# hguo/ftk

Measured on NVIDIA B200. Metric: space_time_simplices_tested_per_sec, higher is better.
Workload: dtype f64+int64

## Files before the change

### ftk_b200/csrc/context.cpp

```cpp
#include <algorithm>
#include <cfloat>
#include <chrono>
#include <cmath>
#include <cstdio>
#include <cstdlib>
#include <cstring>
#include <deque>
#include <string>
#include <thread>
#include <atomic>
#include <vector>

#include <memory>
#include "kernels.h"
#include "online.h"
#include "curves.h"

using namespace ftkb;

namespace {

thread_local std::string g_create_error;

struct Layer {
// ... 593 lines not shown
    c->stats.h2d_bytes += 8 * n;
  }
  return FTKB_OK;
}

static void fill_sweep_geometry(const ftkb_ctx *c, SweepParams &p) {
  p.coords_mode = c->coords_mode;
  p.coords_ncomp = c->coords_ncomp;
  for (int k = 0; k < 6; k++) p.coords_bounds[k] = c->coords_bounds[k];
  p.coords = c->d_coords;
  p.nd = c->n;
  p.sm_count = c->sm_count;
  p.W = c->cfg.dims[0]; p.H = c->cfg.dims[1]; p.D = c->n == 3 ? c->cfg.dims[2] : 1;
  for (int j = 0; j < 3; j++) {
    const bool used = j < c->n;
    p.lb[j] = used ? c->cfg.lb[j] : 0;
    p.ub[j] = used ? c->cfg.ub[j] : 0;
    p.nc[j] = p.ub[j] - p.lb[j] + 1;
    p.vmax[j] = p.ub[j];
    p.voff[j] = 0; p.rank_lb[j] = p.lb[j]; p.rank_nc[j] = p.nc[j];
  }
  for (int j = 0; j < 3; j++)
    p.res_thr[j] = res_threshold_key(c->resolution, c->n == 2 ? (double)(c->cfg.dims[j < 2 ? j : 0] - 1) : 0.5);
  if (c->slab) {
    p.voff[2] = c->cfg.slab_offset;
    p.rank_lb[2] = c->cfg.slab_global_lb;
    p.rank_nc[2] = c->cfg.slab_global_ub - c->cfg.slab_global_lb + 1;
  }
}

static void fused2d_decomposition(const ftkb_ctx *c, SweepParams &p, bool aligned) {
  if (aligned) {
    const int R = SCAN2D_CELL_ROWS;
    p.nsx = std::max(1, (p.W + 7 * 62 - 1) / (7 * 62));
    const int64_t want = std::max<int64_t>(1, (8 * (int64_t)c->sm_count * 3) / p.nsx);
    p.rows = std::max(2 * R, (int)((p.H + want - 1) / want));
    p.rows = (p.rows + R - 1) / R * R;
    p.rows = std::min(p.rows, 64 * R);
  } else {
    p.nsx = std::max(1, (p.W - 1 + 59) / 60);
    int64_t nsy = (2 * (int64_t)c->sm_count * 2 * 8) / p.nsx;
    nsy = std::max<int64_t>(1, std::min<int64_t>(nsy, (p.H + 31) / 32));
    p.rows = (int)((p.H + nsy - 1) / nsy);
  }
  p.nsy = (p.H + p.rows - 1) / p.rows;
  p.nsz = 1;
}

static void fused3d_decomposition(const ftkb_ctx *c, SweepParams &p) {
  p.nsx = (p.W + F3_STRIDE - 1) / F3_STRIDE;
  p.nsy = (p.H + F3_TROWS - 1) / F3_TROWS;
  const int64_t tiles = (int64_t)p.nsx * p.nsy;
  const int64_t slots = 2 * (int64_t)c->sm_count;
  const int64_t nsz = std::max<int64_t>(1, std::min<int64_t>((6 * slots + tiles - 1) / tiles, std::max(1, p.D / 16)));
  p.rows = (int)((p.D + nsz - 1) / nsz);
  p.rows = std::min(p.rows, 63);
  p.nsz = (p.D + p.rows - 1) / p.rows;
}

static void vcells_decomposition(const ftkb_ctx *c, SweepParams &p) {
  if (c->n == 3) { fused3d_decomposition(c, p); return; }
  const int R = VSCAN2D_CELL_ROWS;
  p.nsx = std::max(1, (p.W + 61) / 62);
  const int64_t want = std::max<int64_t>(1, (6 * (int64_t)c->sm_count * 16) / p.nsx);
  p.rows = std::max(2 * R, (int)((p.H + want - 1) / want));
  p.rows = (p.rows + R - 1) / R * R;
  p.nsy = (p.H + p.rows - 1) / p.rows;
// ... 1314 lines not shown
```

### ftk_b200/csrc/kernels.cu

```cuda
#include "kernels.h"

#include <algorithm>
#include <cfloat>
#include <cstdlib>
#include <string>
#include <climits>
#include <cub/device/device_radix_sort.cuh>
#include <cub/device/device_select.cuh>

namespace ftkb {

typedef long long i64;
typedef unsigned long long u64;

__constant__ DeviceMeshTables c_mesh[2];

void upload_mesh_tables(const DeviceMeshTables &t2, const DeviceMeshTables &t3) {
  DeviceMeshTables h[2] = {t2, t3};
  cudaMemcpyToSymbol(c_mesh, h, sizeof(h));
}

constexpr int KEY_ONE = 0x3FF00000;
constexpr int KEY_POISON_EXP = 0x43E00000;

// ... 342 lines not shown
  const int lane = threadIdx.x & 31;
  const i64 warp = (i64)blockIdx.x * (blockDim.x >> 5) + (threadIdx.x >> 5);
  const int sx = (int)(warp % p.nsx), cy = (int)(warp / p.nsx);
  if (cy >= p.nsy) return;
  const int b = sx * 60;
  if (b == 0 || b + 65 > p.W) fused2d_strip<HAS_NEXT, true>(p, b, cy, lane);
  else fused2d_strip<HAS_NEXT, false>(p, b, cy, lane);
}

constexpr int FB_SEG = 68;
constexpr int FB_STRIDE = 62;

__device__ __forceinline__ uint32_t smem_u32(const void *q) { return (uint32_t)__cvta_generic_to_shared(q); }
__device__ __forceinline__ void mbar_init(uint32_t bar, uint32_t count) {
  asm volatile("mbarrier.init.shared::cta.b64 [%0], %1;" ::"r"(bar), "r"(count) : "memory");
}
__device__ __forceinline__ void mbar_expect_tx(uint32_t bar, uint32_t bytes) {
  asm volatile("mbarrier.arrive.expect_tx.shared::cta.b64 _, [%0], %1;" ::"r"(bar), "r"(bytes) : "memory");
}
__device__ __forceinline__ void bulk_g2s(uint32_t dst, const void *src, uint32_t bytes, uint32_t bar) {
  asm volatile("cp.async.bulk.shared::cluster.global.mbarrier::complete_tx::bytes [%0], [%1], %2, [%3];"
               ::"r"(dst), "l"(src), "r"(bytes), "r"(bar) : "memory");
}
__device__ __forceinline__ void mbar_wait(uint32_t bar, uint32_t parity) {
  uint32_t done;
  do {
    asm volatile("{\n\t.reg .pred p;\n\tmbarrier.try_wait.parity.shared::cta.b64 p, [%1], %2;\n\tselp.u32 %0, 1, 0, p;\n\t}"
                 : "=r"(done) : "r"(bar), "r"(parity) : "memory");
  } while (!done);
}
__device__ __forceinline__ void mbar_arrive(uint32_t bar) {
  asm volatile("mbarrier.arrive.shared::cta.b64 _, [%0];" ::"r"(bar) : "memory");
}

__device__ __forceinline__ void tma_load_3d(uint32_t dst, const CUtensorMap *tm, int c0, int c1, int c2, uint32_t bar) {
  asm volatile("cp.async.bulk.tensor.3d.shared::cluster.global.tile.mbarrier::complete_tx::bytes [%0], [%1, {%2, %3, %4}], [%5];"
               ::"r"(dst), "l"(tm), "r"(c0), "r"(c1), "r"(c2), "r"(bar) : "memory");
}

template <int K> struct IC { static constexpr int value = K; };

__device__ __forceinline__ bool elect_one() {
  uint32_t pred;
  asm volatile("{\n\t.reg .pred p;\n\telect.sync _|p, 0xffffffff;\n\tselp.u32 %0, 1, 0, p;\n\t}" : "=r"(pred));
  return pred != 0;
}

__device__ __forceinline__ void res_update4(double &m, float &mf, bool e_in, bool o_in, double dxe, double dye, double dxo, double dyo, double cw, double ch) {
  const double vxe = dxe * cw, vye = dye * ch, vxo = dxo * cw, vyo = dyo * ch;
  if (e_in) {
    if (vxe != 0.0 && fabs(vxe) < fabs(m)) m = vxe;
    if (vye != 0.0 && fabs(vye) < fabs(m)) m = vye;
  }
  if (o_in) {
    if (vxo != 0.0 && fabs(vxo) < fabs(m)) m = vxo;
    if (vyo != 0.0 && fabs(vyo) < fabs(m)) m = vyo;
  }
  mf = fabs(m) < 1e38 ? __double2float_ru(fabs(m)) * 1.000001f : 3.4028234e38f;
}

constexpr int C2_R = 9;
constexpr int C2_NST = 9;
constexpr int C2_CW = 7;
constexpr int C2_SEG = C2_CW * FB_STRIDE + 8;
static_assert(C2_R % 3 == 0 && C2_R == C2_NST && C2_R == SCAN2D_CELL_ROWS, "row window / ring / cell block must stay aligned");

__device__ __forceinline__ size_t cells2d_index(const SweepParams &p, const int strip, const int kb, const int lane) {
  const size_t nblk = (size_t)(p.H / C2_R + 2);
  return ((size_t)strip * nblk + (size_t)kb) * 32u + (size_t)lane;
}

template <int NL>
__device__ __forceinline__ void cells2d_slow_cubes_t(const SweepParams &p, unsigned failmask, const int c0, const int y0, const uint32_t stage) {
  static_assert(2 * C2_R <= 32, "one lane per cube");
  const int W = p.W, H = p.H;
  const int lane = threadIdx.x & 31;
  const float cwf = (float)(W - 1), chf = (float)(H - 1);
  const float nanf_ = __int_as_float(0x7FC00000);
  const int per = 2 * C2_R, total = per * __popc(failmask);
  for (int q0 = 0; q0 < total; q0 += 32) {
    const int qi = q0 + lane;
    const bool live = qi < total;
    const int which = live ? qi / per : 0, within = live ? qi % per : 0;
    const int src = (int)__fns(failmask, 0, which + 1);
    const int r = within >> 1, q = within & 1;
    const int x = c0 + 2 * src + q, y = y0 + r;
    const bool in = live && x >= p.lb[0] && x <= p.ub[0] && y >= p.lb[1] && y <= p.ub[1];
    const int xs[4] = {clampi(x - 1, W), clampi(x, W), clampi(x + 1, W), clampi(x + 2, W)};
    size_t rows_[4];
#pragma unroll
    for (int k = 0; k < 4; k++) rows_[k] = (size_t)W * (size_t)clampi(y - 1 + k, H);
    FRange rx{nanf_, nanf_}, ry{nanf_, nanf_};
#pragma unroll
    for (int L = 0; L < NL; L++) {
      const double *S = p.L[L].S;
      double h[2][4], lo[2], hi[2];
#pragma unroll
      for (int j = 0; j < 2; j++)
#pragma unroll
        for (int k = 0; k < 4; k++) h[j][k] = __ldg(S + rows_[1 + j] + xs[k]);
#pragma unroll
      for (int i = 0; i < 2; i++) { lo[i] = __ldg(S + rows_[0] + xs[1 + i]); hi[i] = __ldg(S + rows_[3] + xs[1 + i]); }
#pragma unroll
      for (int v = 0; v < 4; v++) {
        const int i = v & 1, j = v >> 1;
        if (!in || x + i > p.ub[0] || y + j > p.ub[1]) continue;
        const double dx = h[j][i + 2] - h[j][i];
        const double dy = (j == 0 ? h[1][i + 1] : hi[i]) - (j == 0 ? lo[i] : h[0][i + 1]);
        const float fx = __double2float_rn(dx) * cwf, fy = __double2float_rn(dy) * chf;
        rx = fmerge(rx, FRange{fx, fx}); ry = fmerge(ry, FRange{fy, fy});
      }
    }
    const bool surv = in && !cube_excluded2_f(rx, ry, p.thrp_f, p.thr2_f, p.lim_f);
    const u64 lin = (u64)(x - p.lb[0]) + (u64)p.nc[0] * (u64)(y - p.lb[1]);
    if (stage) stage_survivors(p, stage, surv, lin);
    else append_survivors(p, surv, lin);
  }
}
__device__ __noinline__ void cells2d_slow_cubes(const SweepParams &p, unsigned failmask, const int c0, const int y0, const int nl, const uint32_t stage = 0) {
  if (nl == 1) cells2d_slow_cubes_t<1>(p, failmask, c0, y0, stage);
  else cells2d_slow_cubes_t<2>(p, failmask, c0, y0, stage);
}

__device__ __forceinline__ void cells2d_decide(const SweepParams &p, const FRange ux, const FRange uy, const bool own, const int e, const int y0, const int nl) {
  const bool fail = own && !cube_excluded2_f(ux, uy, p.thrp_f, p.thr2_f, p.lim_f);
  const unsigned fm = __ballot_sync(0xffffffffu, fail);
  if (fm) cells2d_slow_cubes(p, fm, e - 2 * (int)(threadIdx.x & 31), y0, nl);
}

template <bool BORDER, int NPREV, bool TEST>
__device__ __forceinline__ void cells2d_strip(const SweepParams &p, const int c0, const int r0, const int r1, const int lane,
                                              const double *tile , const uint32_t full0, const uint32_t empty0,
                                              const int strip) {
  const int W = p.W, H = p.H, B = p.build_layer;
  const int e = c0 + 2 * lane, o = e + 1;
  const bool e_in = !BORDER || e < W, o_in = !BORDER || o < W, o1_in = !BORDER || o + 1 < W;
  const bool own_cols = lane <= 30 && ((e >= p.lb[0] && e <= p.ub[0]) || (o >= p.lb[0] && o <= p.ub[0]));
  const int jl = r1 + 1;
  const float cwf = (float)(W - 1), chf = (float)(H - 1);
  const bool want_res = p.res_slot[B] != nullptr;
  double rmin = DBL_MAX;
  float rminf = 3.4028234e38f;
  const uint4 *sum_prev = NPREV ? p.sum_in[0] + cells2d_index(p, strip, 0, lane) : nullptr;
  uint4 *sum_out = p.sum_out + cells2d_index(p, strip, 0, lane);

  const double *lane_base = tile + 2 * lane;
  auto centre = [&](const int st, double (&dst)[2]) {
    const double2 t = *reinterpret_cast<const double2 *>(lane_base + st * C2_SEG + 2);
    dst[0] = t.x; dst[1] = t.y;
  };
  auto release = [&](const int st) {
    __syncwarp();
    if (elect_one()) mbar_arrive(empty0 + 8u * st);
  };
  auto finish_block = [&](const int kb, FRange bx, FRange by, const uint4 prevc) {
    bx = fmerge(bx, fshfl_down1(bx));
    by = fmerge(by, fshfl_down1(by));
    sum_out[(size_t)kb * 32u] = make_uint4(__float_as_uint(bx.mn), __float_as_uint(bx.mx), __float_as_uint(by.mn), __float_as_uint(by.mx));
    if (TEST) {
      if (NPREV) {
        bx = fmerge(bx, FRange{__uint_as_float(prevc.x), __uint_as_float(prevc.y)});
        by = fmerge(by, FRange{__uint_as_float(prevc.z), __uint_as_float(prevc.w)});
      }
      const int y0 = kb * C2_R;
      const bool own = own_cols && y0 <= p.ub[1] && y0 + C2_R - 1 >= p.lb[1];
      cells2d_decide(p, bx, by, own, e, y0, NPREV + 1);
    }
  };

  double win[3][2];
  mbar_wait(full0, 0);
  centre(0, win[0]);
  mbar_wait(full0 + 8, 0);
  centre(1, win[1]);
  release(0);
  FRange bx{0.f, 0.f}, by{0.f, 0.f};
  uint4 prevc = make_uint4(0x7FC00000u, 0x7FC00000u, 0x7FC00000u, 0x7FC00000u);

  auto step = [&](auto KC, const int j, const int i) {
    constexpr int K = decltype(KC)::value;
    constexpr int ST_J = (1 + K) % C2_NST, ST_P = (2 + K) % C2_NST;
    double (&m1)[2] = win[K % 3];
    double (&c0v)[2] = win[(K + 1) % 3];
    double (&p1)[2] = win[(K + 2) % 3];
    mbar_wait(full0 + 8u * ST_P, (uint32_t)((i + (2 + K >= C2_NST ? 1 : 0)) & 1));
    centre(ST_P, p1);
    const double *rowj = lane_base + ST_J * C2_SEG;
    double left = rowj[1], right = rowj[4];
    double mid_e = c0v[1];
    if (BORDER) {
      if (e == 0) left = c0v[0];
      if (!o_in) mid_e = c0v[0];
      if (!o1_in) right = c0v[1];
    }
    const double dxe = mid_e - left, dxo = right - c0v[0], dye = p1[0] - m1[0], dyo = p1[1] - m1[1];
    const float fxe = __double2float_rn(dxe) * cwf, fxo = __double2float_rn(dxo) * cwf;
    const float fye = __double2float_rn(dye) * chf, fyo = __double2float_rn(dyo) * chf;
    if (want_res && j < H) {
      float a = fminf(fminf(fabsf(fxe), fabsf(fye)), fminf(fabsf(fxo), fabsf(fyo)));
      if (BORDER) a = fminf(e_in ? fminf(fabsf(fxe), fabsf(fye)) : 3.4028234e38f, o_in ? fminf(fabsf(fxo), fabsf(fyo)) : 3.4028234e38f);
      if (a < rminf) res_update4(rmin, rminf, e_in, o_in, dxe, dye, dxo, dyo, (double)(W - 1), (double)(H - 1));
    }
    const FRange rx{fminf(fxe, fxo), fmaxf(fxe, fxo)}, ry{fminf(fye, fyo), fmaxf(fye, fyo)};
    if (K == 0) {
      if (j > r0) finish_block(j / C2_R - 1, fmerge(bx, rx), fmerge(by, ry), prevc);
      bx = rx; by = ry;
      if (NPREV && j < jl) prevc = __ldg(sum_prev + (size_t)(j / C2_R) * 32u);
    } else {
      bx = fmerge(bx, rx); by = fmerge(by, ry);
    }
    release(ST_J);
  };

  for (int j = r0, i = 0; j <= jl; j += C2_NST, i++) {
    step(IC<0>{}, j, i);
    if (j + 1 <= jl) step(IC<1>{}, j + 1, i);
    if (j + 2 <= jl) step(IC<2>{}, j + 2, i);
    if (j + 3 <= jl) step(IC<3>{}, j + 3, i);
    if (j + 4 <= jl) step(IC<4>{}, j + 4, i);
    if (j + 5 <= jl) step(IC<5>{}, j + 5, i);
    if (j + 6 <= jl) step(IC<6>{}, j + 6, i);
    if (j + 7 <= jl) step(IC<7>{}, j + 7, i);
    if (j + 8 <= jl) step(IC<8>{}, j + 8, i);
  }
  if (jl % C2_R != 0) finish_block(jl / C2_R, bx, by, prevc);
  if (want_res) warp_res_commit(fabs(rmin), p.res_slot[B]);
}

template <int NPREV, bool TEST>
__global__ void __launch_bounds__((C2_CW + 1) * 32, 3) scan2d_build_kernel(const __grid_constant__ SweepParams p) {
  constexpr uint32_t STAGE_BYTES = C2_SEG * 8;
  extern __shared__ __align__(128) unsigned char fb_smem[];
  const int lane = threadIdx.x & 31;
  const int wib = __shfl_sync(0xffffffffu, (int)(threadIdx.x >> 5), 0);
  double *ring = reinterpret_cast<double *>(fb_smem);
  const uint32_t full0 = smem_u32(fb_smem + (size_t)C2_NST * STAGE_BYTES), empty0 = full0 + 8u * C2_NST;
  const int W = p.W, H = p.H;
  const int bx = blockIdx.x % p.nsx, cy = blockIdx.x / p.nsx;
  const int C0 = bx * (C2_CW * FB_STRIDE);
  const int nactive = min(C2_CW, (W - C0 + FB_STRIDE - 1) / FB_STRIDE);
  if (threadIdx.x == 0) {
#pragma unroll
    for (int q = 0; q < C2_NST; q++) { mbar_init(full0 + 8u * q, 1); mbar_init(empty0 + 8u * q, (uint32_t)nactive); }
    asm volatile("fence.mbarrier_init.release.cluster;" ::: "memory");
    asm volatile("fence.proxy.async.shared::cta;" ::: "memory");
  }
  __syncthreads();
  const int r0 = cy * p.rows;
  const int r1 = min(r0 + p.rows - 1, H - 1);
  const int nrows = (r1 + 1) - r0 + 3;
  if (wib == C2_CW) {
    if (elect_one()) {
      const double *S = p.L[p.build_layer].S;
      const int col_lo = max(C0 - 2, 0), col_hi = min(C0 - 2 + C2_SEG, W);
      const uint32_t seg_bytes = (uint32_t)(col_hi - col_lo) * 8u;
      const uint32_t dst0 = smem_u32(ring) + (uint32_t)(col_lo - (C0 - 2)) * 8u;
      for (int rr = 0; rr < nrows; rr++) {
        const int st = rr % C2_NST;
        if (rr >= C2_NST) mbar_wait(empty0 + 8u * st, (uint32_t)((rr / C2_NST - 1) & 1));
        const size_t off = (size_t)W * (size_t)clampi(r0 - 1 + rr, H) + (size_t)col_lo;
        mbar_expect_tx(full0 + 8u * st, seg_bytes);
        bulk_g2s(dst0 + (uint32_t)st * STAGE_BYTES, S + off, seg_bytes, full0 + 8u * st);
      }
    }
    return;
  }
  if (wib >= nactive) return;
  const int c0 = C0 + wib * FB_STRIDE;
  const double *tile = ring + wib * FB_STRIDE;
  const bool border = c0 == 0 || c0 + FB_SEG - 2 > W;
  if (border) cells2d_strip<true, NPREV, TEST>(p, c0, r0, r1, lane, tile, full0, empty0, bx * C2_CW + wib);
  else cells2d_strip<false, NPREV, TEST>(p, c0, r0, r1, lane, tile, full0, empty0, bx * C2_CW + wib);
}

template <int NL>
__global__ void __launch_bounds__(256) scan2d_cells_kernel(const __grid_constant__ SweepParams p, const int nstrips, const int nblk_used) {
  const int lane = threadIdx.x & 31;
  const long long w = (long long)blockIdx.x * 8 + (threadIdx.x >> 5);
  if (w >= (long long)nstrips * nblk_used) return;
  const int strip = (int)(w / nblk_used), kb = (int)(w % nblk_used);
  const int e = strip * FB_STRIDE + 2 * lane, y0 = kb * C2_R;
  const bool own = lane <= 30 && ((e >= p.lb[0] && e <= p.ub[0]) || (e + 1 >= p.lb[0] && e + 1 <= p.ub[0])) && y0 <= p.ub[1] && y0 + C2_R - 1 >= p.lb[1];
  if (!__any_sync(0xffffffffu, own)) return;
  const float nanf_ = __int_as_float(0x7FC00000);
  FRange ux{nanf_, nanf_}, uy{nanf_, nanf_};
#pragma unroll
  for (int L = 0; L < NL; L++) {
    const uint4 c = __ldg(p.sum_in[L] + cells2d_index(p, strip, kb, lane));
    ux = fmerge(ux, FRange{__uint_as_float(c.x), __uint_as_float(c.y)});
    uy = fmerge(uy, FRange{__uint_as_float(c.z), __uint_as_float(c.w)});
  }
  cells2d_decide(p, ux, uy, own, e, y0, NL);
}

constexpr int K2_R = 3;
constexpr int K2_NST = 4;
constexpr int K2_CTAS = 3;
constexpr uint32_t K2_ROW_BYTES = C2_SEG * 8;
constexpr uint32_t K2_STAGE_BYTES = K2_R * K2_ROW_BYTES;
static_assert(C2_R % K2_R == 0, "cell block = whole stages");

__device__ __forceinline__ double2 lds128_f64(uint32_t a) {
  double2 v;
  asm volatile("ld.shared.v2.f64 {%0, %1}, [%2];" : "=d"(v.x), "=d"(v.y) : "r"(a));
  return v;
}
__device__ __forceinline__ double lds64_f64(uint32_t a) {
  double v;
  asm volatile("ld.shared.f64 %0, [%1];" : "=d"(v) : "r"(a));
  return v;
}
__device__ __forceinline__ void cp_async16(uint32_t dst, const void *src) {
  asm volatile("cp.async.cg.shared.global [%0], [%1], 16;" ::"r"(dst), "l"(src) : "memory");
}
__device__ __forceinline__ void cp_async_wait_all() { asm volatile("cp.async.wait_all;" ::: "memory"); }
__device__ __forceinline__ void cp_async_commit() { asm volatile("cp.async.commit_group;" ::: "memory"); }
template <int N> __device__ __forceinline__ void cp_async_wait_group() { asm volatile("cp.async.wait_group %0;" ::"n"(N) : "memory"); }
__device__ __forceinline__ uint4 lds128_u32(uint32_t a) {
  uint4 v;
  asm volatile("ld.shared.v4.u32 {%0, %1, %2, %3}, [%4];" : "=r"(v.x), "=r"(v.y), "=r"(v.z), "=r"(v.w) : "r"(a) : "memory");
  return v;
}
__device__ __forceinline__ void sts64_f64(uint32_t a, double v) { asm volatile("st.shared.f64 [%0], %1;" ::"r"(a), "d"(v) : "memory"); }
__device__ __forceinline__ float fmax_nan(float a, float b) {
  float r;
  asm("max.NaN.f32 %0, %1, %2;" : "=f"(r) : "f"(a), "f"(b));
  return r;
}

__device__ __forceinline__ double nzmin(double m, double d) {
  double r;
  asm("{\n\t.reg .pred p, q;\n\t.reg .f64 ad, am;\n\tabs.f64 ad, %2;\n\tabs.f64 am, %1;\n\t"
      "setp.neu.f64 q, %2, 0d0000000000000000;\n\tsetp.lt.and.f64 p, ad, am, q;\n\tselp.f64 %0, %2, %1, p;\n\t}"
      : "=d"(r) : "d"(m), "d"(d));
  return r;
}

__device__ __forceinline__ FRange k2_vrange(float kmn, float kmx, double c) {
  const int a = __float_as_int(kmn), b = __float_as_int(kmx);
  const double lo = __hiloint2double(a < 0 ? a + 1 : a, 0);
  const double hi = __hiloint2double(b < 0 ? b : b + 1, 0);
  return FRange{__double2float_rd(lo * c), __double2float_ru(hi * c)};
}

__device__ __forceinline__ void prefetch_l2(const void *q) { asm volatile("prefetch.global.L2 [%0];" ::"l"(q)); }

struct K2Acc { double mdx, mdy; float big; };

template <bool BORDER, int NPREV, bool TEST>
__device__ __forceinline__ K2Acc keys2d_strip(const SweepParams &p, const int c0, const int r0, const int r1, const int lane,
                                           const uint32_t tile_u32 ,
                                           const uint32_t full0, const uint32_t empty0, const int strip,
                                           const uint32_t sbase ,
                                           const uint32_t res_u32 ,
                                           const uint32_t wl_stage ,
                                           const uint32_t cell_stage ,
                                           const K2Acc acc) {
  float big = acc.big;
  const int W = p.W, H = p.H, B = p.build_layer;
  const int e = c0 + 2 * lane, o = e + 1;
  const bool e_in = !BORDER || e < W, o_in = !BORDER || o < W, o1_in = !BORDER || o + 1 < W;
  const bool own_cols = lane <= 30 && ((e >= p.lb[0] && e <= p.ub[0]) || (o >= p.lb[0] && o <= p.ub[0]));
  const int jl = r1 + 1;
  const int nrows = jl - r0 + 1;
  const int ngroups = (nrows + K2_R - 1) / K2_R, nstages = (nrows + 2 + K2_R - 1) / K2_R;
  const double cw = (double)(W - 1), ch = (double)(H - 1);
  const bool want_res = p.res_slot[B] != nullptr;
  const float thrx = p.res_thr[0], thry = p.res_thr[1];
  const uint4 *sum_prev = NPREV ? p.sum_in[0] + cells2d_index(p, strip, 0, lane) : nullptr;
  uint4 *sum_out = p.sum_out + cells2d_index(p, strip, 0, lane);
  const uint32_t lane_u32 = tile_u32 + (uint32_t)lane * 16u;
  const int kb0 = r0 / C2_R;
  unsigned long long failbits = 0;
  const int kb_end = ((r1 + 1) + C2_R - 1) / C2_R;

  auto finish_block = [&](const int kb, float xmn, float xmx, float ymn, float ymx) {
    xmn = fminf(xmn, __shfl_down_sync(0xffffffffu, xmn, 1)); xmx = fmaxf(xmx, __shfl_down_sync(0xffffffffu, xmx, 1));
    ymn = fminf(ymn, __shfl_down_sync(0xffffffffu, ymn, 1)); ymx = fmaxf(ymx, __shfl_down_sync(0xffffffffu, ymx, 1));
    FRange bx = k2_vrange(xmn, xmx, cw), by = k2_vrange(ymn, ymx, ch);
    sum_out[(size_t)kb * 32u] = make_uint4(__float_as_uint(bx.mn), __float_as_uint(bx.mx), __float_as_uint(by.mn), __float_as_uint(by.mx));
    if (TEST) {
      if (NPREV && kb < kb_end) {
        cp_async_wait_all();
        const uint4 prevc = lds128_u32(cell_stage + ((uint32_t)kb & 1u) * 512u);
        bx = fmerge(bx, FRange{__uint_as_float(prevc.x), __uint_as_float(prevc.y)});
        by = fmerge(by, FRange{__uint_as_float(prevc.z), __uint_as_float(prevc.w)});
      }
      const int y0 = kb * C2_R;
      const bool own = own_cols && y0 <= p.ub[1] && y0 + C2_R - 1 >= p.lb[1];
      if (own && !cube_excluded2_f(bx, by, p.thrp_f, p.thr2_f, p.lim_f)) failbits |= 1ull << (kb - kb0);
    }
  };

  double C[2][K2_R][2];
  float KX[2][K2_R][2];
  auto load_stage = [&](auto PC, const int s) {
    constexpr int P = decltype(PC)::value;
    const uint32_t gs = sbase + (uint32_t)s, slot = gs % K2_NST;
    mbar_wait(full0 + 8u * slot, (gs / K2_NST) & 1u);
    const uint32_t base = lane_u32 + slot * K2_STAGE_BYTES;
    double nl[K2_R], nr[K2_R];
#pragma unroll
    for (int i = 0; i < K2_R; i++) {
      const double2 c = lds128_f64(base + (uint32_t)i * K2_ROW_BYTES + 16u);
      C[P][i][0] = c.x; C[P][i][1] = c.y;
      nl[i] = lds64_f64(base + (uint32_t)i * K2_ROW_BYTES + 8u);
      nr[i] = lds64_f64(base + (uint32_t)i * K2_ROW_BYTES + 32u);
    }
    float ax = __int_as_float(0x7F800000);
#pragma unroll
    for (int i = 0; i < K2_R; i++) {
      const float ke = fabsf(hikey(C[P][i][0])), ko = fabsf(hikey(C[P][i][1]));
      big = fmax_nan(big, BORDER ? (e_in ? ke : 0.f) : ke);
      big = fmax_nan(big, BORDER ? (o_in ? ko : 0.f) : ko);
      double left = nl[i], right = nr[i], mid_e = C[P][i][1];
      if (BORDER) {
        if (e == 0) left = C[P][i][0];
        if (!o_in) mid_e = C[P][i][0];
        if (!o1_in) right = C[P][i][1];
      }
      const double dxe = mid_e - left, dxo = right - C[P][i][0];
      KX[P][i][0] = hikey(dxe); KX[P][i][1] = hikey(dxo);
      ax = fminf(ax, fminf(fabsf(KX[P][i][0]), fabsf(KX[P][i][1])));
    }
    if (want_res && __any_sync(0xffffffffu, ax <= thrx)) {
      double mdx = lds64_f64(res_u32);
#pragma unroll
      for (int i = 0; i < K2_R; i++) {
        const int j = r0 + K2_R * s + i - 1;
        if (j >= r0 && j <= jl && j < H) {
          double left = lds64_f64(base + (uint32_t)i * K2_ROW_BYTES + 8u), right = lds64_f64(base + (uint32_t)i * K2_ROW_BYTES + 32u), mid_e = C[P][i][1];
          if (BORDER) {
            if (e == 0) left = C[P][i][0];
            if (!o_in) mid_e = C[P][i][0];
            if (!o1_in) right = C[P][i][1];
          }
          if (e_in) mdx = nzmin(mdx, mid_e - left);
          if (o_in) mdx = nzmin(mdx, right - C[P][i][0]);
        }
      }
      sts64_f64(res_u32, mdx);
    }
    __syncwarp();
    if (elect_one()) mbar_arrive(empty0 + 8u * slot);
  };

  float bxmn = 0.f, bxmx = 0.f, bymn = 0.f, bymx = 0.f;
  const uint4 nanc = make_uint4(0x7FC00000u, 0x7FC00000u, 0x7FC00000u, 0x7FC00000u);
  int kb = r0 / C2_R;
  if (NPREV && kb < kb_end) prefetch_l2(sum_prev + (size_t)kb * 32u);
  if (NPREV && kb + 1 < kb_end) prefetch_l2(sum_prev + (size_t)(kb + 1) * 32u);

  int gphase = 0;
  static_assert(C2_R == 3 * K2_R, "a cell block is three groups");
  auto group = [&](auto PC, const int g) {
    constexpr int P = decltype(PC)::value;
    if (g + 1 < nstages) load_stage(IC<1 - P>{}, g + 1);
    const bool opens_group = gphase == 0;
    gphase = gphase == 2 ? 0 : gphase + 1;
    const int j0 = r0 + K2_R * g;
    const bool full = j0 + K2_R - 1 <= min(jl, H - 1);
    float ay = __int_as_float(0x7F800000);
#pragma unroll
    for (int i = 0; i < K2_R; i++) {
      const int j = j0 + i;
      if (!full && j > jl) break;
      const double *m1 = C[P][i];
      const float *kx = i + 1 < K2_R ? KX[P][i + 1] : KX[1 - P][i + 1 - K2_R];
      const double *p1 = i + 2 < K2_R ? C[P][i + 2] : C[1 - P][i + 2 - K2_R];
      const double dye = p1[0] - m1[0], dyo = p1[1] - m1[1];
      const float kxe = kx[0], kxo = kx[1], kye = hikey(dye), kyo = hikey(dyo);
      ay = fminf(ay, fminf(fabsf(kye), fabsf(kyo)));
      if (i == 0 && opens_group) {
        const float rxmn = fminf(kxe, kxo), rxmx = fmaxf(kxe, kxo), rymn = fminf(kye, kyo), rymx = fmaxf(kye, kyo);
        if (j > r0) finish_block(kb - 1, fminf(bxmn, rxmn), fmaxf(bxmx, rxmx), fminf(bymn, rymn), fmaxf(bymx, rymx));
        bxmn = rxmn; bxmx = rxmx; bymn = rymn; bymx = rymx;
        if (NPREV && kb < kb_end) cp_async16(cell_stage + ((uint32_t)kb & 1u) * 512u, sum_prev + (size_t)kb * 32u);
// ... 8 lines not shown
      double mdy = lds64_f64(res_u32 + 8u);
#pragma unroll
      for (int i = 0; i < K2_R; i++) {
        const int j = j0 + i;
        if (!full && (j > jl || j >= H)) break;
        const double *m1 = C[P][i];
        const double *p1 = i + 2 < K2_R ? C[P][i + 2] : C[1 - P][i + 2 - K2_R];
        if (e_in) mdy = nzmin(mdy, p1[0] - m1[0]);
        if (o_in) mdy = nzmin(mdy, p1[1] - m1[1]);
      }
      sts64_f64(res_u32 + 8u, mdy);
    }
  };

  load_stage(IC<0>{}, 0);
#pragma unroll 1
  for (int g = 0; g < ngroups; g += 2) {
    group(IC<0>{}, g);
    if (g + 1 < ngroups) group(IC<1>{}, g + 1);
  }
  if (jl % C2_R != 0) finish_block(jl / C2_R, bxmn, bxmx, bymn, bymx);
  if (TEST) {
    for (int b = 0; b < 64; b++) {
      if (!__any_sync(0xffffffffu, (failbits >> b) != 0)) break;
      const unsigned fm = __ballot_sync(0xffffffffu, (failbits >> b) & 1ull);
      if (fm) cells2d_slow_cubes(p, fm, c0, (kb0 + b) * C2_R, NPREV + 1, wl_stage);
    }
    flush_survivors(p, wl_stage);
  }
  return K2Acc{lds64_f64(res_u32), lds64_f64(res_u32 + 8u), big};
}

template <int NPREV, bool TEST>
__global__ void __launch_bounds__((C2_CW + 1) * 32, K2_CTAS) scan2d_keys_build_kernel(const __grid_constant__ SweepParams p) {
  extern __shared__ __align__(128) unsigned char fb_smem[];
  const int lane = threadIdx.x & 31;
  const int wib = __shfl_sync(0xffffffffu, (int)(threadIdx.x >> 5), 0);
  const uint32_t ring0 = smem_u32(fb_smem);
  const uint32_t full0 = ring0 + (uint32_t)K2_NST * K2_STAGE_BYTES, empty0 = full0 + 8u * K2_NST;
  const uint32_t res_u32 = empty0 + 8u * K2_NST + 16u * threadIdx.x;
  const uint32_t wl_stage = empty0 + 8u * K2_NST + 16u * (C2_CW + 1) * 32u + 32u + WL_STAGE_BYTES * (uint32_t)wib;
  const uint32_t cell_stage = empty0 + 8u * K2_NST + 16u * (C2_CW + 1) * 32u + 32u + WL_STAGE_BYTES * (uint32_t)C2_CW + 1024u * (uint32_t)wib + 16u * (uint32_t)lane;
  const int W = p.W, H = p.H;
  const int bx = blockIdx.x % p.nsx, cy = blockIdx.x / p.nsx;
  const int C0 = bx * (C2_CW * FB_STRIDE);
  const int nactive = min(C2_CW, (W - C0 + FB_STRIDE - 1) / FB_STRIDE);
  if (threadIdx.x == 0) {
#pragma unroll
    for (int q = 0; q < K2_NST; q++) { mbar_init(full0 + 8u * q, 1); mbar_init(empty0 + 8u * q, (uint32_t)nactive); }
    asm volatile("fence.mbarrier_init.release.cluster;" ::: "memory");
    asm volatile("fence.proxy.async.shared::cta;" ::: "memory");
  }
  __syncthreads();
  const int r0 = cy * p.rows;
  const int r1 = min(r0 + p.rows - 1, H - 1);
  const int nstages = ((r1 + 1) - r0 + 1 + 2 + K2_R - 1) / K2_R;
  if (wib == C2_CW) {
    if (elect_one()) {
      const double *S = p.L[p.build_layer].S;
      const int col_lo = max(C0 - 2, 0), col_hi = min(C0 - 2 + C2_SEG, W);
      const uint32_t seg_bytes = (uint32_t)(col_hi - col_lo) * 8u;
      const uint32_t dst0 = ring0 + (uint32_t)(col_lo - (C0 - 2)) * 8u;
      for (int s = 0; s < nstages; s++) {
        const uint32_t slot = (uint32_t)s % K2_NST;
        if (s >= K2_NST) mbar_wait(empty0 + 8u * slot, (uint32_t)((s / K2_NST - 1) & 1));
        mbar_expect_tx(full0 + 8u * slot, seg_bytes * K2_R);
#pragma unroll
        for (int i = 0; i < K2_R; i++) {
          const size_t off = (size_t)W * (size_t)clampi(r0 - 1 + K2_R * s + i, H) + (size_t)col_lo;
          bulk_g2s(dst0 + slot * K2_STAGE_BYTES + (uint32_t)i * K2_ROW_BYTES, S + off, seg_bytes, full0 + 8u * slot);
        }
      }
    }
    return;
  }
  if (wib >= nactive) return;
  const int c0 = C0 + wib * FB_STRIDE;
  const uint32_t tile_u32 = ring0 + (uint32_t)(wib * FB_STRIDE) * 8u;
  const bool border = c0 == 0 || c0 + FB_SEG - 2 > W;
  K2Acc acc{DBL_MAX, DBL_MAX, 0.f};
  sts64_f64(res_u32, DBL_MAX); sts64_f64(res_u32 + 8u, DBL_MAX);
  if (lane == 0) asm volatile("st.shared.s32 [%0], %1;" ::"r"(wl_stage), "r"(0) : "memory");
  __syncwarp();
  if (border) acc = keys2d_strip<true, NPREV, TEST>(p, c0, r0, r1, lane, tile_u32, full0, empty0, bx * C2_CW + wib, 0u, res_u32, wl_stage, cell_stage, acc);
  else acc = keys2d_strip<false, NPREV, TEST>(p, c0, r0, r1, lane, tile_u32, full0, empty0, bx * C2_CW + wib, 0u, res_u32, wl_stage, cell_stage, acc);
  if (p.res_slot[p.build_layer] != nullptr) {
    const double cw = (double)(W - 1), ch = (double)(H - 1);
    const double ax = fabs(acc.mdx), ay = fabs(acc.mdy);
    const double vx = ax < DBL_MAX ? ax * cw : DBL_MAX, vy = ay < DBL_MAX ? ay * ch : DBL_MAX;
    warp_res_commit(fmin(vx > 0.0 ? vx : DBL_MAX, vy > 0.0 ? vy : DBL_MAX), p.res_slot[p.build_layer]);
  }
  if (!(acc.big < __int_as_float(KEYF_BIG))) atomicExch(p.poison, 1ull);
}

static size_t k2_smem_bytes() { return (size_t)K2_NST * K2_STAGE_BYTES + (size_t)2 * K2_NST * 8 + (size_t)16 * (C2_CW + 1) * 32 + 32 + (size_t)WL_STAGE_BYTES * C2_CW + (size_t)1024 * C2_CW; }
static size_t c2_smem_bytes() { return (size_t)C2_NST * C2_SEG * 8 + (size_t)2 * C2_NST * 8; }

size_t scan2d_cells_per_layer(const SweepParams &p) {
  return (size_t)p.nsx * C2_CW * (size_t)(p.H / C2_R + 2) * 32u;
}

void launch_scan2d_cells(const SweepParams &p, cudaStream_t s) {
  const unsigned grid = (unsigned)((i64)p.nsx * p.nsy);
  const int nstrips = (p.W + FB_STRIDE - 1) / FB_STRIDE, nblk = (p.H + C2_R - 1) / C2_R;
  const unsigned tgrid = (unsigned)(((i64)nstrips * nblk + 7) / 8);
  if (p.keys2d && p.sum_mode <= SUM_BUILD_TEST2) {
    switch (p.sum_mode) {
      case SUM_BUILD: scan2d_keys_build_kernel<0, false><<<grid, (C2_CW + 1) * 32, k2_smem_bytes(), s>>>(p); break;
      case SUM_BUILD_TEST1: scan2d_keys_build_kernel<0, true><<<grid, (C2_CW + 1) * 32, k2_smem_bytes(), s>>>(p); break;
      default: scan2d_keys_build_kernel<1, true><<<grid, (C2_CW + 1) * 32, k2_smem_bytes(), s>>>(p); break;
    }
    return;
  }
  switch (p.sum_mode) {
    case SUM_BUILD: scan2d_build_kernel<0, false><<<grid, (C2_CW + 1) * 32, c2_smem_bytes(), s>>>(p); break;
    case SUM_BUILD_TEST1: scan2d_build_kernel<0, true><<<grid, (C2_CW + 1) * 32, c2_smem_bytes(), s>>>(p); break;
    case SUM_BUILD_TEST2: scan2d_build_kernel<1, true><<<grid, (C2_CW + 1) * 32, c2_smem_bytes(), s>>>(p); break;
    case SUM_TEST1: scan2d_cells_kernel<1><<<tgrid, 256, 0, s>>>(p, nstrips, nblk); break;
    default: scan2d_cells_kernel<2><<<tgrid, 256, 0, s>>>(p, nstrips, nblk); break;
  }
}

constexpr int F3_LAYER_BYTES = ((F3_ROWS * F3_COLS * 8 + 127) / 128) * 128;
constexpr uint32_t F3_BOX_BYTES = F3_ROWS * F3_COLS * 8;

__device__ __noinline__ void fused3d_slow_cubes(const SweepParams &p, unsigned failmask, const int C0, const int y0, const int z, const int nl) {
  static_assert(2 * F3_RW * 4 == 32, "four lanes per cube");
  const int lane = threadIdx.x & 31;
  const bool vec = !p.fused;
  const int nbits20 = (p.nbits - (vec ? 0 : 1)) << 20;
  const size_t sy = (size_t)p.W, sz = (size_t)p.W * (size_t)p.H;
  const int cube = lane >> 2, sub = lane & 3;
  const int r = cube >> 1, q = cube & 1;
  while (failmask) {
    const int src = __ffs(failmask) - 1;
    failmask &= failmask - 1;
    const int x = C0 + 2 * src + q, y = y0 + r;
    const bool in = x >= p.lb[0] && x <= p.ub[0] && y >= p.lb[1] && y <= p.ub[1];
    KeyRange rg[3] = {neutral_range(), neutral_range(), neutral_range()};
#pragma unroll
    for (int vv = 0; vv < 2; vv++) {
      const int v = 2 * sub + vv;
      const int vx = x + (v & 1), vy = y + ((v >> 1) & 1), vz = z + (v >> 2);
      if (!in || vx > p.ub[0] || vy > p.ub[1] || vz > p.ub[2]) continue;
      const bool border = vx < 1 || vx > p.W - 2 || vy < 1 || vy > p.H - 2 || vz < 1 || vz > p.D - 2;
      const size_t idx = (size_t)vx + sy * (size_t)vy + sz * (size_t)vz;
      for (int L = 0; L < nl; L++) {
        const double *S = p.L[L].S;
        int h0 = 0, h1 = 0, h2 = 0;
        if (vec) {
// ... 1862 lines not shown
```

Baseline: 5631 billion.

## Drop dedicated TMA producer warp; last consumer warp refills ring stage

```diff
diff --git a/ftk_b200/csrc/context.cpp b/ftk_b200/csrc/context.cpp
--- a/ftk_b200/csrc/context.cpp
+++ b/ftk_b200/csrc/context.cpp
@@ -649,7 +649,7 @@
 static void fused2d_decomposition(const ftkb_ctx *c, SweepParams &p, bool aligned) {
   if (aligned) {
     const int R = SCAN2D_CELL_ROWS;
-    p.nsx = std::max(1, (p.W + 7 * 62 - 1) / (7 * 62));
+    p.nsx = std::max(1, (p.W + 8 * 62 - 1) / (8 * 62));
     const int64_t want = std::max<int64_t>(1, (8 * (int64_t)c->sm_count * 3) / p.nsx);
     p.rows = std::max(2 * R, (int)((p.H + want - 1) / want));
     p.rows = (p.rows + R - 1) / R * R;
diff --git a/ftk_b200/csrc/kernels.cu b/ftk_b200/csrc/kernels.cu
--- a/ftk_b200/csrc/kernels.cu
+++ b/ftk_b200/csrc/kernels.cu
@@ -398,6 +398,14 @@
 __device__ __forceinline__ void mbar_arrive(uint32_t bar) {
   asm volatile("mbarrier.arrive.shared::cta.b64 _, [%0];" ::"r"(bar) : "memory");
 }
+__device__ __forceinline__ bool stage_release_last(uint32_t empty, uint32_t cnt, uint32_t n, uint32_t parity) {
+  mbar_arrive(empty);
+  uint32_t old;
+  asm volatile("atom.relaxed.cta.shared.inc.u32 %0, [%1], %2;" : "=r"(old) : "r"(cnt), "r"(n - 1u) : "memory");
+  if (old != n - 1u) return false;
+  mbar_wait(empty, parity);
+  return true;
+}
 
 __device__ __forceinline__ void tma_load_3d(uint32_t dst, const CUtensorMap *tm, int c0, int c1, int c2, uint32_t bar) {
   asm volatile("cp.async.bulk.tensor.3d.shared::cluster.global.tile.mbarrier::complete_tx::bytes [%0], [%1, {%2, %3, %4}], [%5];"
@@ -405,12 +413,6 @@
 }
 
 template <int K> struct IC { static constexpr int value = K; };
-
-__device__ __forceinline__ bool elect_one() {
-  uint32_t pred;
-  asm volatile("{\n\t.reg .pred p;\n\telect.sync _|p, 0xffffffff;\n\tselp.u32 %0, 1, 0, p;\n\t}" : "=r"(pred));
-  return pred != 0;
-}
 
 __device__ __forceinline__ void res_update4(double &m, float &mf, bool e_in, bool o_in, double dxe, double dye, double dxo, double dyo, double cw, double ch) {
   const double vxe = dxe * cw, vye = dye * ch, vxo = dxo * cw, vyo = dyo * ch;
@@ -427,13 +429,28 @@
 
 constexpr int C2_R = 9;
 constexpr int C2_NST = 9;
-constexpr int C2_CW = 7;
+constexpr int C2_CW = 8;
 constexpr int C2_SEG = C2_CW * FB_STRIDE + 8;
 static_assert(C2_R % 3 == 0 && C2_R == C2_NST && C2_R == SCAN2D_CELL_ROWS, "row window / ring / cell block must stay aligned");
 
 __device__ __forceinline__ size_t cells2d_index(const SweepParams &p, const int strip, const int kb, const int lane) {
   const size_t nblk = (size_t)(p.H / C2_R + 2);
   return ((size_t)strip * nblk + (size_t)kb) * 32u + (size_t)lane;
+}
+
+template <int R, int NST>
+__device__ __forceinline__ void c2_issue_stage(const SweepParams &p, const uint32_t ring0, const uint32_t full0, const int C0, const int r0, const int s) {
+  constexpr uint32_t ROW_BYTES = C2_SEG * 8;
+  const int W = p.W, H = p.H;
+  const double *S = p.L[p.build_layer].S;
+  const int col_lo = max(C0 - 2, 0), col_hi = min(C0 - 2 + C2_SEG, W);
+  const uint32_t seg_bytes = (uint32_t)(col_hi - col_lo) * 8u;
+  const uint32_t slot = (uint32_t)s % NST, bar = full0 + 8u * slot;
+  const uint32_t dst = ring0 + slot * (R * ROW_BYTES) + (uint32_t)(col_lo - (C0 - 2)) * 8u;
+  mbar_expect_tx(bar, seg_bytes * R);
+#pragma unroll
+  for (int i = 0; i < R; i++)
+    bulk_g2s(dst + (uint32_t)i * ROW_BYTES, S + (size_t)W * (size_t)clampi(r0 - 1 + R * s + i, H) + (size_t)col_lo, seg_bytes, bar);
 }
 
 template <int NL>
@@ -496,13 +513,15 @@
 
 template <bool BORDER, int NPREV, bool TEST>
 __device__ __forceinline__ void cells2d_strip(const SweepParams &p, const int c0, const int r0, const int r1, const int lane,
-                                              const double *tile , const uint32_t full0, const uint32_t empty0,
-                                              const int strip) {
+                                              const uint32_t ring0, const double *tile , const uint32_t full0,
+                                              const uint32_t empty0 ,
+                                              const int C0 , const int nactive, const int strip) {
   const int W = p.W, H = p.H, B = p.build_layer;
   const int e = c0 + 2 * lane, o = e + 1;
   const bool e_in = !BORDER || e < W, o_in = !BORDER || o < W, o1_in = !BORDER || o + 1 < W;
   const bool own_cols = lane <= 30 && ((e >= p.lb[0] && e <= p.ub[0]) || (o >= p.lb[0] && o <= p.ub[0]));
   const int jl = r1 + 1;
+  const int nrows = (r1 + 1) - r0 + 3;
   const float cwf = (float)(W - 1), chf = (float)(H - 1);
   const bool want_res = p.res_slot[B] != nullptr;
   double rmin = DBL_MAX;
@@ -515,9 +534,12 @@
     const double2 t = *reinterpret_cast<const double2 *>(lane_base + st * C2_SEG + 2);
     dst[0] = t.x; dst[1] = t.y;
   };
-  auto release = [&](const int st) {
+  auto release = [&](const int st, const int q) {
     __syncwarp();
-    if (elect_one()) mbar_arrive(empty0 + 8u * st);
+    if (lane == 0 && stage_release_last(empty0 + 8u * (uint32_t)st, empty0 + 8u * C2_NST + 4u * (uint32_t)st, (uint32_t)nactive, (uint32_t)(q / C2_NST) & 1u) &&
+        q + C2_NST < nrows) {
+      c2_issue_stage<1, C2_NST>(p, ring0, full0, C0, r0, q + C2_NST);
+    }
   };
   auto finish_block = [&](const int kb, FRange bx, FRange by, const uint4 prevc) {
     bx = fmerge(bx, fshfl_down1(bx));
@@ -539,7 +561,7 @@
   centre(0, win[0]);
   mbar_wait(full0 + 8, 0);
   centre(1, win[1]);
-  release(0);
+  release(0, 0);
   FRange bx{0.f, 0.f}, by{0.f, 0.f};
   uint4 prevc = make_uint4(0x7FC00000u, 0x7FC00000u, 0x7FC00000u, 0x7FC00000u);
 
@@ -575,7 +597,7 @@
     } else {
       bx = fmerge(bx, rx); by = fmerge(by, ry);
     }
-    release(ST_J);
+    release(ST_J, j - r0 + 1);
   };
 
   for (int j = r0, i = 0; j <= jl; j += C2_NST, i++) {
@@ -594,49 +616,38 @@
 }
 
 template <int NPREV, bool TEST>
-__global__ void __launch_bounds__((C2_CW + 1) * 32, 3) scan2d_build_kernel(const __grid_constant__ SweepParams p) {
-  constexpr uint32_t STAGE_BYTES = C2_SEG * 8;
+__global__ void __launch_bounds__(C2_CW * 32, 3) scan2d_build_kernel(const __grid_constant__ SweepParams p) {
   extern __shared__ __align__(128) unsigned char fb_smem[];
   const int lane = threadIdx.x & 31;
   const int wib = __shfl_sync(0xffffffffu, (int)(threadIdx.x >> 5), 0);
-  double *ring = reinterpret_cast<double *>(fb_smem);
-  const uint32_t full0 = smem_u32(fb_smem + (size_t)C2_NST * STAGE_BYTES), empty0 = full0 + 8u * C2_NST;
+  const double *ring = reinterpret_cast<const double *>(fb_smem);
+  const uint32_t ring0 = smem_u32(fb_smem);
+  const uint32_t full0 = ring0 + (uint32_t)C2_NST * C2_SEG * 8u, empty0 = full0 + 8u * C2_NST;
   const int W = p.W, H = p.H;
   const int bx = blockIdx.x % p.nsx, cy = blockIdx.x / p.nsx;
   const int C0 = bx * (C2_CW * FB_STRIDE);
   const int nactive = min(C2_CW, (W - C0 + FB_STRIDE - 1) / FB_STRIDE);
+  const int r0 = cy * p.rows;
+  const int r1 = min(r0 + p.rows - 1, H - 1);
   if (threadIdx.x == 0) {
 #pragma unroll
-    for (int q = 0; q < C2_NST; q++) { mbar_init(full0 + 8u * q, 1); mbar_init(empty0 + 8u * q, (uint32_t)nactive); }
+    for (int q = 0; q < C2_NST; q++) {
+      mbar_init(full0 + 8u * q, 1);
+      mbar_init(empty0 + 8u * q, (uint32_t)nactive);
+      asm volatile("st.shared.u32 [%0], %1;" ::"r"(empty0 + 8u * C2_NST + 4u * q), "r"(0u) : "memory");
+    }
     asm volatile("fence.mbarrier_init.release.cluster;" ::: "memory");
     asm volatile("fence.proxy.async.shared::cta;" ::: "memory");
+    const int nrows = (r1 + 1) - r0 + 3;
+    for (int q = 0; q < min(C2_NST, nrows); q++) c2_issue_stage<1, C2_NST>(p, ring0, full0, C0, r0, q);
   }
   __syncthreads();
-  const int r0 = cy * p.rows;
-  const int r1 = min(r0 + p.rows - 1, H - 1);
-  const int nrows = (r1 + 1) - r0 + 3;
-  if (wib == C2_CW) {
-    if (elect_one()) {
-      const double *S = p.L[p.build_layer].S;
-      const int col_lo = max(C0 - 2, 0), col_hi = min(C0 - 2 + C2_SEG, W);
-      const uint32_t seg_bytes = (uint32_t)(col_hi - col_lo) * 8u;
-      const uint32_t dst0 = smem_u32(ring) + (uint32_t)(col_lo - (C0 - 2)) * 8u;
-      for (int rr = 0; rr < nrows; rr++) {
-        const int st = rr % C2_NST;
-        if (rr >= C2_NST) mbar_wait(empty0 + 8u * st, (uint32_t)((rr / C2_NST - 1) & 1));
-        const size_t off = (size_t)W * (size_t)clampi(r0 - 1 + rr, H) + (size_t)col_lo;
-        mbar_expect_tx(full0 + 8u * st, seg_bytes);
-        bulk_g2s(dst0 + (uint32_t)st * STAGE_BYTES, S + off, seg_bytes, full0 + 8u * st);
-      }
-    }
-    return;
-  }
   if (wib >= nactive) return;
   const int c0 = C0 + wib * FB_STRIDE;
   const double *tile = ring + wib * FB_STRIDE;
   const bool border = c0 == 0 || c0 + FB_SEG - 2 > W;
-  if (border) cells2d_strip<true, NPREV, TEST>(p, c0, r0, r1, lane, tile, full0, empty0, bx * C2_CW + wib);
-  else cells2d_strip<false, NPREV, TEST>(p, c0, r0, r1, lane, tile, full0, empty0, bx * C2_CW + wib);
+  if (border) cells2d_strip<true, NPREV, TEST>(p, c0, r0, r1, lane, ring0, tile, full0, empty0, C0, nactive, bx * C2_CW + wib);
+  else cells2d_strip<false, NPREV, TEST>(p, c0, r0, r1, lane, ring0, tile, full0, empty0, C0, nactive, bx * C2_CW + wib);
 }
 
 template <int NL>
@@ -666,6 +677,7 @@
 constexpr uint32_t K2_STAGE_BYTES = K2_R * K2_ROW_BYTES;
 static_assert(C2_R % K2_R == 0, "cell block = whole stages");
 
+
 __device__ __forceinline__ double2 lds128_f64(uint32_t a) {
   double2 v;
   asm volatile("ld.shared.v2.f64 {%0, %1}, [%2];" : "=d"(v.x), "=d"(v.y) : "r"(a));
@@ -715,9 +727,9 @@
 
 template <bool BORDER, int NPREV, bool TEST>
 __device__ __forceinline__ K2Acc keys2d_strip(const SweepParams &p, const int c0, const int r0, const int r1, const int lane,
-                                           const uint32_t tile_u32 ,
-                                           const uint32_t full0, const uint32_t empty0, const int strip,
-                                           const uint32_t sbase ,
+                                           const uint32_t ring0, const uint32_t tile_u32 ,
+                                           const uint32_t full0, const uint32_t empty0 ,
+                                           const int C0 , const int nactive, const int strip,
                                            const uint32_t res_u32 ,
                                            const uint32_t wl_stage ,
                                            const uint32_t cell_stage ,
@@ -762,8 +774,8 @@
   float KX[2][K2_R][2];
   auto load_stage = [&](auto PC, const int s) {
     constexpr int P = decltype(PC)::value;
-    const uint32_t gs = sbase + (uint32_t)s, slot = gs % K2_NST;
-    mbar_wait(full0 + 8u * slot, (gs / K2_NST) & 1u);
+    const uint32_t slot = (uint32_t)s % K2_NST;
+    mbar_wait(full0 + 8u * slot, ((uint32_t)s / K2_NST) & 1u);
     const uint32_t base = lane_u32 + slot * K2_STAGE_BYTES;
     double nl[K2_R], nr[K2_R];
 #pragma unroll
@@ -808,7 +820,10 @@
       sts64_f64(res_u32, mdx);
     }
     __syncwarp();
-    if (elect_one()) mbar_arrive(empty0 + 8u * slot);
+    if (lane == 0 && stage_release_last(empty0 + 8u * slot, empty0 + 8u * K2_NST + 4u * slot, (uint32_t)nactive, ((uint32_t)s / K2_NST) & 1u) &&
+        s + K2_NST < nstages) {
+      c2_issue_stage<K2_R, K2_NST>(p, ring0, full0, C0, r0, s + K2_NST);
+    }
   };
 
   float bxmn = 0.f, bxmx = 0.f, bymn = 0.f, bymx = 0.f;
@@ -883,48 +898,34 @@
 }
 
 template <int NPREV, bool TEST>
-__global__ void __launch_bounds__((C2_CW + 1) * 32, K2_CTAS) scan2d_keys_build_kernel(const __grid_constant__ SweepParams p) {
+__global__ void __launch_bounds__(C2_CW * 32, K2_CTAS) scan2d_keys_build_kernel(const __grid_constant__ SweepParams p) {
   extern __shared__ __align__(128) unsigned char fb_smem[];
   const int lane = threadIdx.x & 31;
   const int wib = __shfl_sync(0xffffffffu, (int)(threadIdx.x >> 5), 0);
   const uint32_t ring0 = smem_u32(fb_smem);
-  const uint32_t full0 = ring0 + (uint32_t)K2_NST * K2_STAGE_BYTES, empty0 = full0 + 8u * K2_NST;
-  const uint32_t res_u32 = empty0 + 8u * K2_NST + 16u * threadIdx.x;
-  const uint32_t wl_stage = empty0 + 8u * K2_NST + 16u * (C2_CW + 1) * 32u + 32u + WL_STAGE_BYTES * (uint32_t)wib;
-  const uint32_t cell_stage = empty0 + 8u * K2_NST + 16u * (C2_CW + 1) * 32u + 32u + WL_STAGE_BYTES * (uint32_t)C2_CW + 1024u * (uint32_t)wib + 16u * (uint32_t)lane;
+  const uint32_t full0 = ring0 + (uint32_t)K2_NST * K2_STAGE_BYTES, empty0 = full0 + 8u * K2_NST, cnt0 = empty0 + 8u * K2_NST;
+  const uint32_t res_u32 = cnt0 + 8u * K2_NST + 16u * threadIdx.x;
+  const uint32_t wl_stage = cnt0 + 8u * K2_NST + 16u * C2_CW * 32u + 32u + WL_STAGE_BYTES * (uint32_t)wib;
+  const uint32_t cell_stage = cnt0 + 8u * K2_NST + 16u * C2_CW * 32u + 32u + WL_STAGE_BYTES * (uint32_t)C2_CW + 1024u * (uint32_t)wib + 16u * (uint32_t)lane;
   const int W = p.W, H = p.H;
   const int bx = blockIdx.x % p.nsx, cy = blockIdx.x / p.nsx;
   const int C0 = bx * (C2_CW * FB_STRIDE);
   const int nactive = min(C2_CW, (W - C0 + FB_STRIDE - 1) / FB_STRIDE);
+  const int r0 = cy * p.rows;
+  const int r1 = min(r0 + p.rows - 1, H - 1);
   if (threadIdx.x == 0) {
 #pragma unroll
-    for (int q = 0; q < K2_NST; q++) { mbar_init(full0 + 8u * q, 1); mbar_init(empty0 + 8u * q, (uint32_t)nactive); }
+    for (int q = 0; q < K2_NST; q++) {
+      mbar_init(full0 + 8u * q, 1);
+      mbar_init(empty0 + 8u * q, (uint32_t)nactive);
+      asm volatile("st.shared.u32 [%0], %1;" ::"r"(cnt0 + 4u * q), "r"(0u) : "memory");
+    }
     asm volatile("fence.mbarrier_init.release.cluster;" ::: "memory");
     asm volatile("fence.proxy.async.shared::cta;" ::: "memory");
+    const int nstages = ((r1 + 1) - r0 + 1 + 2 + K2_R - 1) / K2_R;
+    for (int s = 0; s < min(K2_NST, nstages); s++) c2_issue_stage<K2_R, K2_NST>(p, ring0, full0, C0, r0, s);
   }
   __syncthreads();
-  const int r0 = cy * p.rows;
-  const int r1 = min(r0 + p.rows - 1, H - 1);
-  const int nstages = ((r1 + 1) - r0 + 1 + 2 + K2_R - 1) / K2_R;
-  if (wib == C2_CW) {
-    if (elect_one()) {
-      const double *S = p.L[p.build_layer].S;
-      const int col_lo = max(C0 - 2, 0), col_hi = min(C0 - 2 + C2_SEG, W);
-      const uint32_t seg_bytes = (uint32_t)(col_hi - col_lo) * 8u;
-      const uint32_t dst0 = ring0 + (uint32_t)(col_lo - (C0 - 2)) * 8u;
-      for (int s = 0; s < nstages; s++) {
-        const uint32_t slot = (uint32_t)s % K2_NST;
-        if (s >= K2_NST) mbar_wait(empty0 + 8u * slot, (uint32_t)((s / K2_NST - 1) & 1));
-        mbar_expect_tx(full0 + 8u * slot, seg_bytes * K2_R);
-#pragma unroll
-        for (int i = 0; i < K2_R; i++) {
-          const size_t off = (size_t)W * (size_t)clampi(r0 - 1 + K2_R * s + i, H) + (size_t)col_lo;
-          bulk_g2s(dst0 + slot * K2_STAGE_BYTES + (uint32_t)i * K2_ROW_BYTES, S + off, seg_bytes, full0 + 8u * slot);
-        }
-      }
-    }
-    return;
-  }
   if (wib >= nactive) return;
   const int c0 = C0 + wib * FB_STRIDE;
   const uint32_t tile_u32 = ring0 + (uint32_t)(wib * FB_STRIDE) * 8u;
@@ -933,8 +934,8 @@
   sts64_f64(res_u32, DBL_MAX); sts64_f64(res_u32 + 8u, DBL_MAX);
   if (lane == 0) asm volatile("st.shared.s32 [%0], %1;" ::"r"(wl_stage), "r"(0) : "memory");
   __syncwarp();
-  if (border) acc = keys2d_strip<true, NPREV, TEST>(p, c0, r0, r1, lane, tile_u32, full0, empty0, bx * C2_CW + wib, 0u, res_u32, wl_stage, cell_stage, acc);
-  else acc = keys2d_strip<false, NPREV, TEST>(p, c0, r0, r1, lane, tile_u32, full0, empty0, bx * C2_CW + wib, 0u, res_u32, wl_stage, cell_stage, acc);
+  if (border) acc = keys2d_strip<true, NPREV, TEST>(p, c0, r0, r1, lane, ring0, tile_u32, full0, empty0, C0, nactive, bx * C2_CW + wib, res_u32, wl_stage, cell_stage, acc);
+  else acc = keys2d_strip<false, NPREV, TEST>(p, c0, r0, r1, lane, ring0, tile_u32, full0, empty0, C0, nactive, bx * C2_CW + wib, res_u32, wl_stage, cell_stage, acc);
   if (p.res_slot[p.build_layer] != nullptr) {
     const double cw = (double)(W - 1), ch = (double)(H - 1);
     const double ax = fabs(acc.mdx), ay = fabs(acc.mdy);
@@ -944,8 +945,8 @@
   if (!(acc.big < __int_as_float(KEYF_BIG))) atomicExch(p.poison, 1ull);
 }
 
-static size_t k2_smem_bytes() { return (size_t)K2_NST * K2_STAGE_BYTES + (size_t)2 * K2_NST * 8 + (size_t)16 * (C2_CW + 1) * 32 + 32 + (size_t)WL_STAGE_BYTES * C2_CW + (size_t)1024 * C2_CW; }
-static size_t c2_smem_bytes() { return (size_t)C2_NST * C2_SEG * 8 + (size_t)2 * C2_NST * 8; }
+static size_t k2_smem_bytes() { return (size_t)K2_NST * K2_STAGE_BYTES + (size_t)3 * K2_NST * 8 + (size_t)16 * C2_CW * 32 + 32 + (size_t)WL_STAGE_BYTES * C2_CW + (size_t)1024 * C2_CW; }
+static size_t c2_smem_bytes() { return (size_t)C2_NST * C2_SEG * 8 + (size_t)2 * C2_NST * 8 + (size_t)C2_NST * 4; }
 
 size_t scan2d_cells_per_layer(const SweepParams &p) {
   return (size_t)p.nsx * C2_CW * (size_t)(p.H / C2_R + 2) * 32u;
@@ -957,16 +958,16 @@
   const unsigned tgrid = (unsigned)(((i64)nstrips * nblk + 7) / 8);
   if (p.keys2d && p.sum_mode <= SUM_BUILD_TEST2) {
     switch (p.sum_mode) {
-      case SUM_BUILD: scan2d_keys_build_kernel<0, false><<<grid, (C2_CW + 1) * 32, k2_smem_bytes(), s>>>(p); break;
-      case SUM_BUILD_TEST1: scan2d_keys_build_kernel<0, true><<<grid, (C2_CW + 1) * 32, k2_smem_bytes(), s>>>(p); break;
-      default: scan2d_keys_build_kernel<1, true><<<grid, (C2_CW + 1) * 32, k2_smem_bytes(), s>>>(p); break;
+      case SUM_BUILD: scan2d_keys_build_kernel<0, false><<<grid, C2_CW * 32, k2_smem_bytes(), s>>>(p); break;
+      case SUM_BUILD_TEST1: scan2d_keys_build_kernel<0, true><<<grid, C2_CW * 32, k2_smem_bytes(), s>>>(p); break;
+      default: scan2d_keys_build_kernel<1, true><<<grid, C2_CW * 32, k2_smem_bytes(), s>>>(p); break;
     }
     return;
   }
   switch (p.sum_mode) {
-    case SUM_BUILD: scan2d_build_kernel<0, false><<<grid, (C2_CW + 1) * 32, c2_smem_bytes(), s>>>(p); break;
-    case SUM_BUILD_TEST1: scan2d_build_kernel<0, true><<<grid, (C2_CW + 1) * 32, c2_smem_bytes(), s>>>(p); break;
-    case SUM_BUILD_TEST2: scan2d_build_kernel<1, true><<<grid, (C2_CW + 1) * 32, c2_smem_bytes(), s>>>(p); break;
+    case SUM_BUILD: scan2d_build_kernel<0, false><<<grid, C2_CW * 32, c2_smem_bytes(), s>>>(p); break;
+    case SUM_BUILD_TEST1: scan2d_build_kernel<0, true><<<grid, C2_CW * 32, c2_smem_bytes(), s>>>(p); break;
+    case SUM_BUILD_TEST2: scan2d_build_kernel<1, true><<<grid, C2_CW * 32, c2_smem_bytes(), s>>>(p); break;
     case SUM_TEST1: scan2d_cells_kernel<1><<<tgrid, 256, 0, s>>>(p, nstrips, nblk); break;
     default: scan2d_cells_kernel<2><<<tgrid, 256, 0, s>>>(p, nstrips, nblk); break;
   }
```

Result: slower. 4750 billion, median of 6 (-15.6%).
